# rehakvoj1/BIH-GPU-Raytracer

Measured on NVIDIA B200. Metric: Mrays/s, higher is better.
Workload: dtype f32

## Files before the change

bih-gpu-raytracer_b200/csrc/trace.cu:

```cuda
#include "bihrt_internal.cuh"
#include <float.h>

#define FULL 0xffffffffu
#define STACK_DEPTH_PARITY  32
#define STACK_DEPTH_QUALITY 96
#define NONE 0xFFFFFFFFu
#ifndef TRACE_THREADS
#define TRACE_THREADS 128
#endif
#ifndef TRACE_MIN_BLOCKS
#define TRACE_MIN_BLOCKS 8
#endif

#ifndef TRACE_COVERAGE_EXIT
#define TRACE_COVERAGE_EXIT 1
#endif
#define BOX_EPS 2.384185791015625e-07f

#define DET_EPS __uint_as_float(0x358637beu)

struct Hit { float t; int slot; };

__device__ __forceinline__ float fmin3(float a, float b, float c) { float r; asm("min.f32 %0, %1, %2, %3;" : "=f"(r) : "f"(a), "f"(b), "f"(c)); return r; }
__device__ __forceinline__ float fmax3(float a, float b, float c) { float r; asm("max.f32 %0, %1, %2, %3;" : "=f"(r) : "f"(a), "f"(b), "f"(c)); return r; }

__device__ __forceinline__ uint32_t pack_colour(uint32_t hits, int samples) {
    const float fh = (float)hits, fm = (float)(samples - (int)hits), fs = (float)samples;
    float cr = __fdiv_rn(__fadd_rn(__fmul_rn(fh, 255.f), __fmul_rn(fm, 20.f)), fs);
    float cb = __fdiv_rn(__fmul_rn(fm, 40.f), fs);
    cr = fmaxf(0.f, fminf(255.f, cr));
    cb = fmaxf(0.f, fminf(255.f, cb));
    return ((uint32_t)(int)cb << 16) | ((uint32_t)(int)cr << 8) | (uint32_t)(int)cr;
}

__device__ __forceinline__ float mt_det(float dx, float dy, float dz, float e1x, float e1y, float e1z, float e2x, float e2y, float e2z,
                                        float& px, float& py, float& pz) {
    px = __fsub_rn(__fmul_rn(dy, e2z), __fmul_rn(e2y, dz));
    py = __fsub_rn(__fmul_rn(dz, e2x), __fmul_rn(e2z, dx));
    pz = __fsub_rn(__fmul_rn(dx, e2y), __fmul_rn(e2x, dy));
    return __fadd_rn(__fadd_rn(__fmul_rn(e1x, px), __fmul_rn(e1y, py)), __fmul_rn(e1z, pz));
}
__device__ __forceinline__ float mt_u(float ox, float oy, float oz, const float4& q0, float px, float py, float pz, float inv,
                                      float& tx, float& ty, float& tz) {
    tx = __fsub_rn(ox, q0.x); ty = __fsub_rn(oy, q0.y); tz = __fsub_rn(oz, q0.z);
    return __fmul_rn(__fadd_rn(__fadd_rn(__fmul_rn(tx, px), __fmul_rn(ty, py)), __fmul_rn(tz, pz)), inv);
}
__device__ __forceinline__ float mt_v(float dx, float dy, float dz, float e1x, float e1y, float e1z, float tx, float ty, float tz, float inv,
                                      float& qx, float& qy, float& qz) {
    qx = __fsub_rn(__fmul_rn(ty, e1z), __fmul_rn(e1y, tz));
    qy = __fsub_rn(__fmul_rn(tz, e1x), __fmul_rn(e1z, tx));
    qz = __fsub_rn(__fmul_rn(tx, e1y), __fmul_rn(e1x, ty));
    return __fmul_rn(__fadd_rn(__fadd_rn(__fmul_rn(dx, qx), __fmul_rn(dy, qy)), __fmul_rn(dz, qz)), inv);
}

template <bool COUNTED, bool FIRST, bool RANGE = false, bool TWO_SIDED = false>
__device__ __forceinline__ void test_leaf(const char* __restrict__ first_tri, float ox, float oy, float oz,
                                          float dx, float dy, float dz, Hit& h, uint32_t& ntris, uint32_t& wleaf,
                                          const float* tlo_p = nullptr) {
    const float4* p = reinterpret_cast<const float4*>(first_tri);
    for (;;) {
        const float4 q0 = __ldg(p), q1 = __ldg(p + 1), q2 = __ldg(p + 2);
        if (COUNTED) { ntris++; const uint32_t am = __activemask(); wleaf += ((threadIdx.x & 31) == __ffs(am) - 1); }
        const float e1x = q0.w, e1y = q1.x, e1z = q1.y, e2x = q1.z, e2y = q1.w, e2z = q2.x;
        float px, py, pz;
        const float det = mt_det(dx, dy, dz, e1x, e1y, e1z, e2x, e2y, e2z, px, py, pz);
        if (!((TWO_SIDED ? fabsf(det) : det) < DET_EPS)) {
            const float inv = __frcp_rn(det);
            float tx, ty, tz;
            const float u = mt_u(ox, oy, oz, q0, px, py, pz, inv, tx, ty, tz);
            if (!(u < 0.f || u > 1.f)) {
                float qx, qy, qz;
                const float v = mt_v(dx, dy, dz, e1x, e1y, e1z, tx, ty, tz, inv, qx, qy, qz);
                if (!(v < 0.f || __fadd_rn(u, v) > 1.f)) {
                    const float t = __fmul_rn(__fadd_rn(__fadd_rn(__fmul_rn(e2x, qx), __fmul_rn(e2y, qy)), __fmul_rn(e2z, qz)), inv);
                    if (t > (RANGE ? *tlo_p : 0.f) && t < h.t) {
                        h.t = t; h.slot = (int)__float_as_uint(q2.w);
                        if (FIRST) break;
                    }
                }
            }
        }
        if (__float_as_uint(q2.z) & 1u) break;
        p += 3;
    }
}

template <int MODE, bool COUNTED, int WALK, bool Q>
__global__ void __launch_bounds__(TRACE_THREADS, TRACE_MIN_BLOCKS) k_trace(TraceArgs a) {
    constexpr int STACK_DEPTH = Q ? STACK_DEPTH_QUALITY : STACK_DEPTH_PARITY;
    constexpr bool COVER = MODE == 1 && TRACE_COVERAGE_EXIT != 0;
    constexpr bool LIST = MODE == 0 || MODE == 3 || MODE == 4;
    constexpr bool RANGE = MODE == 3 || MODE == 4;
    constexpr bool TWO_SIDED = MODE == 4;
    __shared__ __align__(16) float s_ray[TRACE_THREADS * 10];
    const int lane = threadIdx.x & 31;
    const uint32_t lt = (1u << lane) - 1u;
    float* my_ray = s_ray + threadIdx.x * 10;
    const char* __restrict__ nodes_b = reinterpret_cast<const char*>(a.nodes);
    const char* __restrict__ tris_b = reinterpret_cast<const char*>(a.tris);
    const BihTri* __restrict__ tris = a.tris;
    const uint32_t nu = a.hdr->nu;
    if (a.hdr->status != 0) return;
    if ((a.hdr->quality != 0) != Q) {
        if (blockIdx.x == 0 && threadIdx.x == 0 && a.status_map) *a.status_map = 0x100u;
        return;
    }
    const float blo[3] = { a.hdr->lo[0], a.hdr->lo[1], a.hdr->lo[2] }, bhi[3] = { a.hdr->hi[0], a.hdr->hi[1], a.hdr->hi[2] };
    uint32_t nnodes = 0, ntris = 0, maxsp = 0;
    uint32_t wnode = 0, wleaf = 0;

    uint64_t total;
    int tx = 1;
    if (LIST) total = a.tile_cost ? (((uint64_t)a.nrays + 1023u) >> 10) << 10 : (uint64_t)a.nrays;
    else {
        tx = (a.w + 31) / 32;
        const int ty = (a.h + 31) / 32, T = tx * ty;
        const int my_tiles = T > a.shard_index ? (T - a.shard_index + a.shard_count - 1) / a.shard_count : 0;
        total = ((uint64_t)my_tiles * 1024u) << a.gshift;
    }
    const int gshift = LIST ? 0 : a.gshift;
    const int nsamp = LIST ? 1 : ((a.s_end - a.s_begin) >> gshift);
    uint32_t my_queue = 0;
    if (a.queues > 1) { asm("mov.u32 %0, %%smid;" : "=r"(my_queue)); my_queue %= (uint32_t)a.queues; }
    uint64_t pool_next = 0, pool_end = 0;
    long long unit_t0 = 0; uint32_t unit_tile = 0xFFFFFFFFu;
    bool exhausted = false;

    uint64_t item = ~0ull;
    int s = 0, s0 = 0;
    uint32_t hits = 0, pixel = 0, pxy = 0;
    float ix = 1.f, iy = 1.f, iz = 1.f, nx = 0.f, ny = 0.f, nz = 0.f, bpad = 0.f;
    uint32_t cur = NONE;
    float rMin = 0.f, pMin = 0.f, pMax = 0.f;
    Hit h; h.t = FLT_MAX; h.slot = -1;
    bool tracing = false;
    uint4 stack[STACK_DEPTH];
    int sp = 0;
#define STACK_RESET() do { sp = 0; } while (0)
#define STACK_PUSH(item) do { stack[sp] = (item); sp++; } while (0)
#define STACK_POP(e) do { sp--; (e) = stack[sp]; } while (0)
    const uint32_t root_ref = BIH_REF_NODE(0, a.hdr->root_axis);
    const bool vote = WALK > 0 || a.vote_wait != 0;
    int thresh = a.refill_threshold;
    const bool direct = MODE == 1 && gshift > 0 && !(a.flags & BIHRT_RENDER_COUNTS);
    if (direct) thresh = 32;
    const int steps_per_vote = WALK > 0 ? WALK : (a.vote_walk > 0 ? a.vote_walk : 1);
    const uint32_t ray_smem = (uint32_t)__cvta_generic_to_shared(my_ray);

    for (;;) {
        const uint32_t idle = __ballot_sync(FULL, cur == NONE);
        const uint32_t busy = ~idle;
        if (idle && (busy == 0 || (thresh < 32 && __popc(__ballot_sync(FULL, cur == NONE && (tracing || item != ~0ull || LIST))) >= thresh))) {
            const bool fresh = (busy == 0);
            int new_thresh = -1;
            bool want_item = false, finishing = false;
            if (cur == NONE) {
                if (tracing) {
                    tracing = false;
                    if (MODE == 1) hits += (h.slot >= 0);
                    else if (RANGE) {
                        const bool hit = h.slot >= 0;
                        const bool rec = a.out_u || a.out_v || a.out_ng;
                        float u = 0.f, v = 0.f, gx = 0.f, gy = 0.f, gz = 0.f;
                        int32_t prim = -1;
                        if (hit && (rec || a.out_prim)) {
                            const float4* tq = reinterpret_cast<const float4*>(tris + h.slot);
                            const float4 q0 = __ldg(tq), q1 = __ldg(tq + 1), q2 = __ldg(tq + 2);
                            prim = (int32_t)__float_as_uint(q2.y);
                            if (rec) {
                                const float e1x = q0.w, e1y = q1.x, e1z = q1.y, e2x = q1.z, e2y = q1.w, e2z = q2.x;
                                const float2 dxy = *reinterpret_cast<const float2*>(my_ray + 6);
                                const float dx = dxy.x, dy = dxy.y, dz = my_ray[8];
                                float px, py, pz, tx, ty, tz, qx, qy, qz;
                                const float inv = __frcp_rn(mt_det(dx, dy, dz, e1x, e1y, e1z, e2x, e2y, e2z, px, py, pz));
                                u = mt_u(my_ray[0], my_ray[2], my_ray[4], q0, px, py, pz, inv, tx, ty, tz);
                                v = mt_v(dx, dy, dz, e1x, e1y, e1z, tx, ty, tz, inv, qx, qy, qz);
                                gx = __fsub_rn(__fmul_rn(e1y, e2z), __fmul_rn(e1z, e2y));
                                gy = __fsub_rn(__fmul_rn(e1z, e2x), __fmul_rn(e1x, e2z));
                                gz = __fsub_rn(__fmul_rn(e1x, e2y), __fmul_rn(e1y, e2x));
                            }
                        }
                        if (a.out_t) a.out_t[item] = hit ? h.t : FLT_MAX;
                        if (a.out_slot) a.out_slot[item] = h.slot;
                        if (a.out_prim) a.out_prim[item] = prim;
                        if (a.out_u) a.out_u[item] = u;
                        if (a.out_v) a.out_v[item] = v;
                        if (a.out_ng) { float* g = a.out_ng + 3 * item; g[0] = gx; g[1] = gy; g[2] = gz; }
                    } else {
                        const uint64_t o = MODE == 0 ? item : (uint64_t)pixel * (uint32_t)a.spp + (uint32_t)(s0 + s);
                        if (a.out_t) a.out_t[o] = h.t;
                        if (a.out_slot) a.out_slot[o] = h.slot;
                        if (a.out_prim) a.out_prim[o] = h.slot >= 0 ? (int32_t)tris[h.slot].prim : -1;
                    }
                    s++;
                    if (s == nsamp) {
                        if (MODE == 1 && gshift > 0) finishing = true;
                        else if (MODE == 1 && (a.flags & BIHRT_RENDER_COUNTS)) a.fb[pixel] = hits;
                        else if (MODE == 1) a.fb[pixel] = pack_colour(hits, nsamp);
                        item = ~0ull;
                    }
                }
                want_item = (item == ~0ull);
            }
            if (MODE == 1 && gshift > 0) {
                const uint32_t fin = __ballot_sync(FULL, finishing);
                if (finishing) {
                    const uint32_t same = __match_any_sync(fin, pixel);
                    const uint32_t sum = __reduce_add_sync(same, hits);
                    if (lane == __ffs(same) - 1) {
                        if (direct) a.fb[pixel] = pack_colour(sum, nsamp << gshift);
                        else if (sum) atomicAdd(&a.fb[pixel], sum);
                    }
                }
            }
            if (!LIST && fresh && a.tile_cost && unit_tile != 0xFFFFFFFFu) {
                if (lane == 0) atomicMax(a.tile_cost + unit_tile, (uint32_t)min((unsigned long long)(clock64() - unit_t0) >> 8, 0xFFFFFFFFull));
                unit_tile = 0xFFFFFFFFu;
            }
            uint32_t want = __ballot_sync(FULL, want_item);
            if (!LIST && busy != 0) want = 0;
            while (want && !exhausted) {
                if (pool_next >= pool_end) {
                    uint64_t base = ~0ull;
                    uint32_t got = 0;
                    if (lane == 0) {
                        const uint32_t ilc = (uint32_t)a.il_count, ili = (uint32_t)a.il_index, ics = (uint32_t)a.il_cshift;
                        if (a.queues <= 1) {
                            const uint32_t chunk = ilc > 1 ? 32u : (uint32_t)a.chunk_items;
                            const uint64_t fetched = atomicAdd(a.work, chunk); got = chunk;
                            const uint64_t lu = fetched >> 5;
                            base = ilc > 1 ? ((((lu >> ics) * ilc + ili) << ics) | (lu & ((1u << ics) - 1u))) << 5 : fetched;
                            if (base >= total) base = ~0ull;
                        } else {
                            const uint32_t tshift = 10 + gshift, ushift = 5 + gshift;
                            const uint64_t ntile = (total + ((1ull << tshift) - 1)) >> tshift;
                            for (uint32_t k = 0; k < (uint32_t)a.queues; k++) {
                                uint32_t q = my_queue + k; if (q >= (uint32_t)a.queues) q -= (uint32_t)a.queues;
                                if (q >= ntile) continue;
                                const uint32_t upt = (1u << ushift) / ilc;
                                const uint64_t units = ((ntile - q + a.queues - 1) / a.queues) * upt;
                                if (ld_relaxed(a.work + q) >= units) continue;
                                const uint32_t u = atomicAdd(a.work + q, 1u);
                                if (u >= units) continue;
                                const uint32_t lu = u % upt;
                                const uint64_t b = (((uint64_t)(u / upt) * a.queues + q) << tshift) + ((uint64_t)((((lu >> ics) * ilc + ili) << ics) | (lu & ((1u << ics) - 1u))) << 5);
                                if (b < total) { base = b; got = 32; break; }
                            }
                        }
                    }
                    base = __shfl_sync(FULL, base, 0);
                    got = __shfl_sync(FULL, got, 0);
                    if (LIST && a.tile_cost && unit_tile != 0xFFFFFFFFu) {
                        if (lane == 0) atomicMax(a.tile_cost + unit_tile, (uint32_t)min((unsigned long long)(clock64() - unit_t0) >> 8, 0xFFFFFFFFull));
                        unit_tile = 0xFFFFFFFFu;
                    }
                    if (base == ~0ull) { exhausted = true; break; }
                    pool_next = base;
                    pool_end = min(base + got, total);
                    if (a.tile_cost && unit_tile == 0xFFFFFFFFu) {
                        const uint32_t m = (uint32_t)(base >> (10 + gshift));
                        unit_tile = a.tile_order ? __ldg(a.tile_order + m) : m;
                        unit_t0 = clock64();
                    }
                }
                const uint64_t avail = pool_end - pool_next;
                const uint32_t rank = __popc(want & lt);
                const bool served = want_item && (uint64_t)rank < avail;
                if (served) {
                    item = pool_next + rank; s = 0; hits = 0; want_item = false;
                    if (LIST && a.tile_cost) {
                        const uint32_t mi = (uint32_t)(item >> 10);
                        const uint64_t ray = ((uint64_t)(a.tile_order ? __ldg(a.tile_order + mi) : mi) << 10) | (item & 1023u);
                        item = ray < (uint64_t)a.nrays ? ray : ~0ull;
                        if (item == ~0ull) want_item = true;
                    }
                    if (MODE == 0 && a.perm && item != ~0ull) item = __ldg(a.perm + item);
                    if (!LIST) {
                        const uint64_t pix = item >> gshift;
                        s0 = a.s_begin + (int)((uint32_t)item & ((1u << gshift) - 1u)) * nsamp;
                        const uint32_t mi = (uint32_t)(pix >> 10), q = (uint32_t)pix & 1023u;
                        const uint32_t m = a.tile_order ? __ldg(a.tile_order + mi) : mi;
                        const int tile = a.shard_index + (int)m * a.shard_count;
                        const int px = (tile % tx) * 32 + (int)((q >> 5) & 3u) * 8 + (int)(q & 7u);
                        const int py = (tile / tx) * 32 + (int)(q >> 7) * 4 + (int)((q >> 3) & 3u);
                        if (px < a.w && py < a.h) { pixel = (uint32_t)(py * a.w + px); pxy = (uint32_t)px | ((uint32_t)py << 16); }
                        else item = ~0ull;
                        if (item == ~0ull) want_item = true;
                    }
                }
                pool_next += min((uint64_t)__popc(want), avail);
                want = __ballot_sync(FULL, want_item);
            }
            if (cur == NONE && item != ~0ull) {
                float ox, oy, oz, dx, dy, dz;
                float tlo = 0.f, thi = FLT_MAX;
                bool live = true;
                if (RANGE) {
                    const float4* p = reinterpret_cast<const float4*>(a.rays_iv + item);
                    const float4 r0 = __ldg(p), r1 = __ldg(p + 1);
                    ox = r0.x; oy = r0.y; oz = r0.z; dx = r1.x; dy = r1.y; dz = r1.z;
                    tlo = fmaxf(r0.w, 0.f);
                    live = r0.w == r0.w && tlo < r1.w;
                    thi = fminf(r1.w, FLT_MAX);
                } else if (MODE == 0) {
                    const float* p = reinterpret_cast<const float*>(a.rays + item);
                    ox = __ldg(p); oy = __ldg(p + 1); oz = __ldg(p + 2); dx = __ldg(p + 3); dy = __ldg(p + 4); dz = __ldg(p + 5);
                } else {
                    const int px = (int)(pxy & 0xFFFFu), py = (int)(pxy >> 16);
                    const float ru = (a.flags & BIHRT_RENDER_JITTER) ? bihrt_jitter(a.seed, pixel, (uint32_t)(s0 + s), 0) : 0.5f;
                    const float rv = (a.flags & BIHRT_RENDER_JITTER) ? bihrt_jitter(a.seed, pixel, (uint32_t)(s0 + s), 1) : 0.5f;
                    const float uu = __fdiv_rn(__fadd_rn((float)px, ru), (float)a.w);
                    const float vv = __fdiv_rn(__fadd_rn((float)py, rv), (float)a.h);
                    ox = a.cam.origin[0]; oy = a.cam.origin[1]; oz = a.cam.origin[2];
                    dx = __fsub_rn(__fadd_rn(__fadd_rn(a.cam.lower_left[0], __fmul_rn(uu, a.cam.horizontal[0])), __fmul_rn(vv, a.cam.vertical[0])), ox);
                    dy = __fsub_rn(__fadd_rn(__fadd_rn(a.cam.lower_left[1], __fmul_rn(uu, a.cam.horizontal[1])), __fmul_rn(vv, a.cam.vertical[1])), oy);
                    dz = __fsub_rn(__fadd_rn(__fadd_rn(a.cam.lower_left[2], __fmul_rn(uu, a.cam.horizontal[2])), __fmul_rn(vv, a.cam.vertical[2])), oz);
                }
                ix = __frcp_rn(dx); iy = __frcp_rn(dy); iz = __frcp_rn(dz);
                nx = -__fmul_rn(ox, ix); ny = -__fmul_rn(oy, iy); nz = -__fmul_rn(oz, iz);
                bpad = __fmul_rn(BOX_EPS, fmaxf(fmaxf(fabsf(nx) <= FLT_MAX ? fabsf(nx) : 0.f, fabsf(ny) <= FLT_MAX ? fabsf(ny) : 0.f),
                                                fabsf(nz) <= FLT_MAX ? fabsf(nz) : 0.f));
                if (LIST && fresh) {
                    const uint32_t m = __activemask();
                    const uint32_t bx = __ballot_sync(m, ix < 0.f), by = __ballot_sync(m, iy < 0.f), bz = __ballot_sync(m, iz < 0.f);
                    const bool mixed = ((bx != 0 && bx != m) + (by != 0 && by != m) + (bz != 0 && bz != m)) >= 2;
                    new_thresh = mixed ? min(a.refill_threshold, a.refill_incoherent) : a.refill_threshold;
                }
                *reinterpret_cast<float2*>(my_ray) = make_float2(ox, ix); *reinterpret_cast<float2*>(my_ray + 2) = make_float2(oy, iy);
                *reinterpret_cast<float2*>(my_ray + 4) = make_float2(oz, iz); *reinterpret_cast<float2*>(my_ray + 6) = make_float2(dx, dy);
                my_ray[8] = dz;
                if (RANGE) my_ray[9] = tlo;
                h.t = RANGE ? thi : (MODE == 0 && a.any_hit) ? a.tmax : FLT_MAX; h.slot = -1; STACK_RESET(); tracing = true;
                bool in = nu > 0 && live;
                float tMin = __fmul_rn(__fsub_rn(ix < 0.f ? bhi[0] : blo[0], ox), ix);
                float tMax = __fmul_rn(__fsub_rn(ix < 0.f ? blo[0] : bhi[0], ox), ix);
                const float tymin = __fmul_rn(__fsub_rn(iy < 0.f ? bhi[1] : blo[1], oy), iy);
                const float tymax = __fmul_rn(__fsub_rn(iy < 0.f ? blo[1] : bhi[1], oy), iy);
                if ((tMin > tymax) || (tymin > tMax)) in = false;
                if (tymin > tMin) tMin = tymin;
                if (tymax < tMax) tMax = tymax;
                const float tzmin = __fmul_rn(__fsub_rn(iz < 0.f ? bhi[2] : blo[2], oz), iz);
                const float tzmax = __fmul_rn(__fsub_rn(iz < 0.f ? blo[2] : bhi[2], oz), iz);
                if ((tMin > tzmax) || (tzmin > tMax)) in = false;
                if (tzmin > tMin) tMin = tzmin;
                if (tzmax < tMax) tMax = tzmax;
                if (in) {
                    const float tabs = fmaxf(fabsf(tMin), fabsf(tMax));
                    bpad = __fmaf_rn(BOX_EPS, tabs <= FLT_MAX ? tabs : FLT_MAX, bpad);
                    const float qnan = __uint_as_float(0x7fc00000u);
                    ix = fabsf(ix) <= FLT_MAX ? ix : qnan; iy = fabsf(iy) <= FLT_MAX ? iy : qnan; iz = fabsf(iz) <= FLT_MAX ? iz : qnan;
                    rMin = tMin; pMin = fmaxf(tMin, tlo); pMax = ((MODE == 0 && a.any_hit) || COVER || RANGE) ? fminf(tMax, h.t) : tMax;
                    if (nu == 1) { cur = BIH_REF_LEAFREF(0); pMin = -FLT_MAX; pMax = FLT_MAX; }
                    else if (pMin <= pMax) cur = root_ref;
                }
            }
            if (LIST) {
                const uint32_t upd = __ballot_sync(FULL, new_thresh >= 0);
                if (upd) thresh = __shfl_sync(FULL, new_thresh, __ffs(upd) - 1);
            }
            if (__ballot_sync(FULL, cur != NONE || tracing) == 0 && exhausted &&
                __ballot_sync(FULL, item != ~0ull) == 0) break;
        }

#define BOX_SLAB(lx, ly, lz, hx, hy, hz, bn, bf)                                                            \
        do {                                                                                                \
            const float ax0 = __fmaf_rn((lx), ix, nx), ax1 = __fmaf_rn((hx), ix, nx);                       \
            const float ay0 = __fmaf_rn((ly), iy, ny), ay1 = __fmaf_rn((hy), iy, ny);                       \
            const float az0 = __fmaf_rn((lz), iz, nz), az1 = __fmaf_rn((hz), iz, nz);                       \
            const float n_ = fmaxf(fmaxf(fminf(ax0, ax1), fminf(ay0, ay1)), fminf(az0, az1));               \
            const float f_ = fminf(fminf(fmaxf(ax0, ax1), fmaxf(ay0, ay1)), fmaxf(az0, az1));               \
            (bn) = __fsub_rn(n_, bpad);                                                                     \
            (bf) = __fadd_rn(f_, bpad);                                                                     \
        } while (0)
#define POP_VALID()                                                                                         \
        do {                                                                                                \
            cur = NONE;                                                                                     \
            if (COVER) {                                   \
                if (sp > 0) {                                                                               \
                    uint4 e;                                                                                \
                    STACK_POP(e);                                                                           \
                    cur = e.x; rMin = __uint_as_float(e.y); pMin = __uint_as_float(e.z); pMax = __uint_as_float(e.w); \
                }                                                                                           \
            } else while (sp > 0) {                                                                         \
                uint4 e;                                                                                    \
                STACK_POP(e);                                                                               \
                const float m = fminf(__uint_as_float(e.w), h.t);                                           \
                if (__uint_as_float(e.z) <= m) { cur = e.x; rMin = __uint_as_float(e.y); pMin = __uint_as_float(e.z); pMax = m; break; } \
            }                                                                                               \
        } while (0)
        for (;;) {
#pragma unroll (WALK > 0 ? WALK : 1)
            for (int rep = 0; rep < steps_per_vote && (int)cur >= 0; rep++) {
                float2 oi;
                uint32_t ra;
                asm("mad.lo.u32 %0, %1, 8, %2;" : "=r"(ra) : "r"(cur & 3u), "r"(ray_smem));
                asm volatile("ld.shared.v2.f32 {%0, %1}, [%2];" : "=f"(oi.x), "=f"(oi.y) : "r"(ra));
                const float4* np;
                asm("mad.wide.u32 %0, %1, 64, %2;" : "=l"(np) : "r"(cur >> 2), "l"(nodes_b));
                float4 nd, b0, b1, b2;
                if (LIST) {
                    asm("ld.global.nc.v8.f32 {%0,%1,%2,%3,%4,%5,%6,%7}, [%8];"
                        : "=f"(nd.x), "=f"(nd.y), "=f"(nd.z), "=f"(nd.w), "=f"(b0.x), "=f"(b0.y), "=f"(b0.z), "=f"(b0.w) : "l"(np));
                    asm("ld.global.nc.v8.f32 {%0,%1,%2,%3,%4,%5,%6,%7}, [%8];"
                        : "=f"(b1.x), "=f"(b1.y), "=f"(b1.z), "=f"(b1.w), "=f"(b2.x), "=f"(b2.y), "=f"(b2.z), "=f"(b2.w) : "l"(np + 2));
                } else { nd = __ldg(np); b0 = __ldg(np + 1); b1 = __ldg(np + 2); b2 = __ldg(np + 3); }
                if (COUNTED) { nnodes++; const uint32_t am = __activemask(); wnode += (lane == __ffs(am) - 1); }
                const uint32_t rl = __float_as_uint(nd.z), rr = __float_as_uint(nd.w);
                const bool neg = oi.y < 0.f;
                const float t0 = __fmul_rn(__fsub_rn(nd.x, oi.x), oi.y);
                const float t1 = __fmul_rn(__fsub_rn(nd.y, oi.x), oi.y);
                const float tn = neg ? t1 : t0, tf = neg ? t0 : t1;
                const uint32_t refn = neg ? rr : rl, reff = neg ? rl : rr;
                float bnL, bfL, bnR, bfR;
                BOX_SLAB(b0.x, b0.y, b0.z, b0.w, b1.x, b1.y, bnL, bfL);
                BOX_SLAB(b1.z, b1.w, b2.x, b2.y, b2.z, b2.w, bnR, bfR);
                const float nLo = fmaxf(pMin, neg ? bnR : bnL), nHi = fmin3(pMax, tn, neg ? bfR : bfL);
                const float fLo = fmax3(pMin, tf, neg ? bnL : bnR), fHi = fminf(pMax, neg ? bfL : bfR);
                const bool go_near = (Q || rMin < tn) && (nLo <= nHi);
                const bool go_far = (fLo <= fHi);
                if (go_near && go_far) {
                    if ((int)refn >= 0 && (int)reff < 0) {
                        STACK_PUSH(make_uint4(refn, __float_as_uint(rMin), __float_as_uint(nLo), __float_as_uint(nHi)));
                        cur = reff; rMin = tf; pMin = fLo; pMax = fHi;
                    } else {
                        STACK_PUSH(make_uint4(reff, __float_as_uint(tf), __float_as_uint(fLo), __float_as_uint(fHi)));
                        cur = refn; pMin = nLo; pMax = nHi;
                    }
                    if (COUNTED) { maxsp = max(maxsp, (uint32_t)sp); if (sp >= STACK_DEPTH) { maxsp = 0x7fffffffu; sp = STACK_DEPTH - 1; } }
#ifdef BIHRT_DEBUG_STACK
                    if (sp >= STACK_DEPTH) __trap();
#endif
                } else if (go_near) { cur = refn; pMin = nLo; pMax = nHi; }
                else if (go_far) { cur = reff; rMin = tf; pMin = fLo; pMax = fHi; }
                else POP_VALID();
            }
            const uint32_t m_walk = __ballot_sync(FULL, (int)cur >= 0);
            if (m_walk == 0) break;
            if (vote) {
                const uint32_t m_wait = __ballot_sync(FULL, cur + 1u > 0x80000000u);
                if (__popc(m_wait) > __popc(m_walk)) break;
            }
        }
        if (cur + 1u > 0x80000000u) {
            const char* tp;
            asm("mad.wide.u32 %0, %1, 12, %2;" : "=l"(tp) : "r"(cur & 0x7FFFFFFCu), "l"(tris_b));
            const float2 dxy = *reinterpret_cast<const float2*>(my_ray + 6);
            test_leaf<COUNTED, COVER, RANGE, TWO_SIDED>(tp, my_ray[0], my_ray[2], my_ray[4], dxy.x, dxy.y, my_ray[8], h, ntris, wleaf, my_ray + 9);
            if (((LIST && a.any_hit) || COVER) && h.slot >= 0) { STACK_RESET(); cur = NONE; }
            else POP_VALID();
        }
#undef POP_VALID
#undef BOX_SLAB
#undef STACK_RESET
#undef STACK_PUSH
#undef STACK_POP
        __syncwarp();
    }

    if (COUNTED) {
#pragma unroll
        for (int o = 16; o > 0; o >>= 1) {
            nnodes += __shfl_xor_sync(FULL, nnodes, o);
            ntris += __shfl_xor_sync(FULL, ntris, o);
            maxsp = max(maxsp, __shfl_xor_sync(FULL, maxsp, o));
        }
        if (lane == 0) {
            atomicAdd(&a.counters[0], (unsigned long long)nnodes);
            atomicAdd(&a.counters[1], (unsigned long long)ntris);
            atomicMax(&a.counters[2], (unsigned long long)maxsp);
        }
        wnode = __reduce_add_sync(FULL, wnode); wleaf = __reduce_add_sync(FULL, wleaf);
        if (lane == 0) { atomicAdd(&a.counters[4], (unsigned long long)wnode); atomicAdd(&a.counters[5], (unsigned long long)wleaf); }
    }
}

__global__ void k_resolve(uint32_t* fb, int npix, int spp) {
    const int i = blockIdx.x * blockDim.x + threadIdx.x;
    if (i >= npix) return;
    fb[i] = pack_colour(fb[i], spp);
}

#define TILE_CLASSES 5
__device__ __forceinline__ int tile_class(uint32_t c, uint32_t mx) {
    int k = 0;
#pragma unroll
    for (int j = 1; j < TILE_CLASSES; j++) k += c < max(1u, mx >> j);
    return k;
}
__global__ void __launch_bounds__(1024) k_tile_order(uint32_t* __restrict__ cost, uint32_t* __restrict__ order, uint32_t ntiles) {
    __shared__ uint32_t s_w[TILE_CLASSES][32];
    __shared__ uint32_t s_max, s_base[TILE_CLASSES];
    const int lane = threadIdx.x & 31, w = threadIdx.x >> 5;
    const uint32_t per = (ntiles + 1023u) / 1024u, i0 = min(ntiles, threadIdx.x * per), i1 = min(ntiles, i0 + per);
    uint32_t mx = 0;
    for (uint32_t i = i0; i < i1; i++) mx = max(mx, cost[i]);
    mx = __reduce_max_sync(0xffffffffu, mx);
    if (lane == 0) s_w[0][w] = mx;
    __syncthreads();
    if (threadIdx.x == 0) { uint32_t m = 0; for (int k = 0; k < 32; k++) m = max(m, s_w[0][k]); s_max = m; }
    __syncthreads();
    mx = s_max;
    uint32_t cnt[TILE_CLASSES], inc[TILE_CLASSES];
#pragma unroll
    for (int k = 0; k < TILE_CLASSES; k++) cnt[k] = 0;
    for (uint32_t i = i0; i < i1; i++) {
        const int cl = tile_class(cost[i], mx);
#pragma unroll
        for (int k = 0; k < TILE_CLASSES; k++) cnt[k] += (cl == k);
    }
    __syncthreads();
#pragma unroll
    for (int k = 0; k < TILE_CLASSES; k++) {
        inc[k] = cnt[k];
#pragma unroll
        for (int o = 1; o < 32; o <<= 1) { const uint32_t t = __shfl_up_sync(0xffffffffu, inc[k], o); if (lane >= o) inc[k] += t; }
        if (lane == 31) s_w[k][w] = inc[k];
    }
    __syncthreads();
    if (threadIdx.x < TILE_CLASSES) {
        uint32_t run = 0;
        for (int j = 0; j < 32; j++) { const uint32_t x = s_w[threadIdx.x][j]; s_w[threadIdx.x][j] = run; run += x; }
        s_base[threadIdx.x] = run;
    }
    __syncthreads();
    if (threadIdx.x == 0) { uint32_t run = 0; for (int k = 0; k < TILE_CLASSES; k++) { const uint32_t x = s_base[k]; s_base[k] = run; run += x; } }
    __syncthreads();
    uint32_t pos[TILE_CLASSES];
#pragma unroll
    for (int k = 0; k < TILE_CLASSES; k++) pos[k] = s_base[k] + s_w[k][w] + inc[k] - cnt[k];
    for (uint32_t i = i0; i < i1; i++) {
        const int cl = tile_class(cost[i], mx);
#pragma unroll
        for (int k = 0; k < TILE_CLASSES; k++) if (cl == k) order[pos[k]++] = i;
    }
    __syncthreads();
    for (uint32_t i = i0; i < i1; i++) cost[i] = 0;
}

__global__ void __launch_bounds__(1024) k_tile_sort(uint32_t* __restrict__ cost, uint32_t* __restrict__ order, uint32_t ntiles) {
    __shared__ uint32_t s_cnt[256], s_off[256];
    if (threadIdx.x < 256) s_cnt[threadIdx.x] = 0;
    __syncthreads();
    for (uint32_t i = threadIdx.x; i < ntiles; i += 1024) atomicAdd(&s_cnt[min(255u, cost[i] >> 4)], 1u);
    __syncthreads();
    if (threadIdx.x == 0) { uint32_t run = 0; for (int b = 255; b >= 0; b--) { s_off[b] = run; run += s_cnt[b]; } }
    __syncthreads();
    for (uint32_t i = threadIdx.x; i < ntiles; i += 1024) order[atomicAdd(&s_off[min(255u, cost[i] >> 4)], 1u)] = i;
    __syncthreads();
    for (uint32_t i = threadIdx.x; i < ntiles; i += 1024) cost[i] = 0;
}

int bihrt_tile_order_launch(bihrt_ctx* c, uint32_t* cost, uint32_t* order, uint32_t ntiles, bool full_sort) {
    if (full_sort) k_tile_sort<<<1, 1024, 0, c->stream>>>(cost, order, ntiles);
    else k_tile_order<<<1, 1024, 0, c->stream>>>(cost, order, ntiles);
    c->kernel_launches += 1;
    BIHRT_CUDA(c, cudaGetLastError());
    return BIHRT_OK;
}

int bihrt_resolve_launch(bihrt_ctx* c, uint32_t* fb, int npix, int spp) {
    k_resolve<<<(npix + 255) / 256, 256, 0, c->stream>>>(fb, npix, spp);
    c->kernel_launches += 1;
    BIHRT_CUDA(c, cudaGetLastError());
    return BIHRT_OK;
}

#ifndef TRACE_WALK
#define TRACE_WALK 4
#endif
template <int MODE, bool COUNTED, int WALK, bool Q = false>
static int launch(bihrt_ctx* c, const TraceArgs& a) {
    int per_sm = c->opt_trace_blocks_per_sm;
    if (per_sm <= 0) {
        BIHRT_CUDA(c, cudaOccupancyMaxActiveBlocksPerMultiprocessor(&per_sm, k_trace<MODE, COUNTED, WALK, Q>, TRACE_THREADS, 0));
        if (per_sm < 1) per_sm = 1;
    }
    BIHRT_CUDA(c, cudaMemsetAsync(a.work, 0, 4 * 1024, c->stream));
    k_trace<MODE, COUNTED, WALK, Q><<<c->sm_count * per_sm, TRACE_THREADS, 0, c->stream>>>(a);
    c->kernel_launches += 1;
    BIHRT_CUDA(c, cudaGetLastError());
    return BIHRT_OK;
}

int bihrt_trace_launch(bihrt_ctx* c, const TraceArgs& a_in, int mode, bool counted) {
    TraceArgs a = a_in;
    const bool list = mode == 0 || mode == 3 || mode == 4;
    const int64_t rays = list ? a.nrays : (int64_t)a.w * a.h * (a.s_end - a.s_begin) / (a.shard_count > 0 ? a.shard_count : 1) / (a.il_count > 0 ? a.il_count : 1);
    const bool on = a.queues < 0 ? (rays >= (16ll << 20) && (list || a.gshift == 0)) : a.queues != 0;
    a.queues = on ? (c->sm_count < 1024 ? c->sm_count : 1024) : 1;
    uint32_t ntiles = 0;
    bihrt_ctx::TileKey key;
    if (!list) {
        const int tx = (a.w + 31) / 32, ty = (a.h + 31) / 32, T = tx * ty;
        const int mine = T > a.shard_index ? (T - a.shard_index + a.shard_count - 1) / a.shard_count : 0;
        if ((((uint64_t)mine * 1024u) << a.gshift) >= (1ull << 32) - (1ull << 24))
            return bihrt_fail(c, BIHRT_ERR_INVALID, "launch of %d tiles x 1024 pixels x %d lane groups exceeds the 32-bit work counter", mine, 1 << a.gshift);
    }
    const bool order_on = a.queues == 1 && (c->opt_tile_order > 1 || (c->opt_tile_order == 1 && rays >= (64ll << 10) && rays < (48ll << 20) && c->n >= 10000));
    if (order_on) {
        if (list) {
            if (a.nrays > 1024 && a.nrays <= (65536ll << 10)) { ntiles = (uint32_t)((a.nrays + 1023) >> 10); key.nrays = a.nrays; }
        } else {
            const int tx = (a.w + 31) / 32, ty = (a.h + 31) / 32, T = tx * ty;
            const int mine = T > a.shard_index ? (T - a.shard_index + a.shard_count - 1) / a.shard_count : 0;
            if (mine > 1 && mine <= 65536) ntiles = (uint32_t)mine;
            key.w = a.w; key.h = a.h; key.gshift = a.gshift; key.nsamp = a.s_end - a.s_begin; key.shard_index = a.shard_index;
            key.shard_count = a.shard_count; key.il_index = a.il_index; key.il_count = a.il_count; key.il_cshift = a.il_cshift;
        }
        key.mode = list ? mode : 1; key.ntiles = ntiles;
    }
    bihrt_ctx::TileSlot* slot = nullptr;
    if (ntiles) {
        for (auto& ts : c->tile_slots) if (ts.cap && ts.key == key) slot = &ts;
        if (!slot) {
            slot = &c->tile_slots[c->tile_next];
            c->tile_next = (c->tile_next + 1) % 4;
            slot->key = key; slot->valid = false;
        }
        if ((size_t)ntiles > slot->cap) {
            if (slot->cost) cudaFree(slot->cost);
            if (slot->order) cudaFree(slot->order);
            slot->cost = slot->order = nullptr; slot->cap = 0; slot->valid = false;
            if (cudaMalloc(&slot->cost, (size_t)ntiles * 4) != cudaSuccess || cudaMalloc(&slot->order, (size_t)ntiles * 4) != cudaSuccess) {
                cudaGetLastError();
                if (slot->cost) { cudaFree(slot->cost); slot->cost = nullptr; }
                slot = nullptr; ntiles = 0;
            } else slot->cap = ntiles;
        }
        if (slot) {
            if (!slot->valid) BIHRT_CUDA(c, cudaMemsetAsync(slot->cost, 0, (size_t)ntiles * 4, c->stream));
            a.tile_cost = slot->cost;
            a.tile_order = slot->valid ? slot->order : nullptr;
        }
    }
    const bool shipped = a.vote_wait != 0 && a.vote_walk == TRACE_WALK;
    int rc = BIHRT_ERR_INVALID;
    a.status_map = c->d_status_map;
    if (c->built_quality) {
        TraceArgs q = a; q.vote_wait = 1; q.vote_walk = 1;
        switch (mode * 2 + (counted ? 1 : 0)) {
            case 0: rc = launch<0, false, TRACE_WALK, true>(c, a); break;
            case 1: rc = launch<0, true, 0, true>(c, q); break;
            case 2: rc = launch<1, false, TRACE_WALK, true>(c, a); break;
            case 3: rc = launch<1, true, 0, true>(c, q); break;
            case 4: rc = launch<2, false, TRACE_WALK, true>(c, a); break;
            case 5: rc = launch<2, true, 0, true>(c, q); break;
            case 6: rc = launch<3, false, TRACE_WALK, true>(c, a); break;
            case 8: rc = launch<4, false, TRACE_WALK, true>(c, a); break;
            default: return bihrt_fail(c, BIHRT_ERR_INVALID, "bad trace mode %d", mode);
        }
    } else
    switch (mode * 2 + (counted ? 1 : 0)) {
        case 0: rc = shipped ? launch<0, false, TRACE_WALK>(c, a) : launch<0, false, 0>(c, a); break;
        case 1: rc = launch<0, true, 0>(c, a); break;
        case 2: rc = shipped ? launch<1, false, TRACE_WALK>(c, a) : launch<1, false, 0>(c, a); break;
        case 3: rc = launch<1, true, 0>(c, a); break;
        case 4: rc = shipped ? launch<2, false, TRACE_WALK>(c, a) : launch<2, false, 0>(c, a); break;
        case 5: rc = launch<2, true, 0>(c, a); break;
        case 6: rc = shipped ? launch<3, false, TRACE_WALK>(c, a) : launch<3, false, 0>(c, a); break;
        case 8: rc = shipped ? launch<4, false, TRACE_WALK>(c, a) : launch<4, false, 0>(c, a); break;
        default: return bihrt_fail(c, BIHRT_ERR_INVALID, "bad trace mode %d", mode);
    }
    if (rc == BIHRT_OK && slot) {
        if ((rc = bihrt_tile_order_launch(c, slot->cost, slot->order, ntiles, rays < c->opt_tile_sort_below)) == BIHRT_OK) slot->valid = true;
    }
    return rc;
}
```

Baseline: 13720.

## Specialize node traversal per warp-uniform ray octant in coverage mode

In coverage mode (MODE 1), each warp checks with ballots whether all its active rays share a direction-sign octant. It stores that octant in shared memory and then runs a node-walk loop instantiated for that octant. In the specialised loop the slab test picks near and far planes directly with 3-input min/max instead of per-axis min/max, which cuts ALU work per box. The cost is six extra ballots per refill, eight more copies of the traversal loop (more code and instruction-cache pressure), and a fallback path for warps with mixed octants.

```diff
diff --git a/bih-gpu-raytracer_b200/csrc/trace.cu b/bih-gpu-raytracer_b200/csrc/trace.cu
--- a/bih-gpu-raytracer_b200/csrc/trace.cu
+++ b/bih-gpu-raytracer_b200/csrc/trace.cu
@@ -15,6 +15,10 @@
 #ifndef TRACE_COVERAGE_EXIT
 #define TRACE_COVERAGE_EXIT 1
 #endif
+#ifndef TRACE_OCTANT_WALK
+#define TRACE_OCTANT_WALK 1
+#endif
+#define OCT_MIXED 8
 #define BOX_EPS 2.384185791015625e-07f
 
 #define DET_EPS __uint_as_float(0x358637beu)
@@ -89,6 +93,7 @@
 __global__ void __launch_bounds__(TRACE_THREADS, TRACE_MIN_BLOCKS) k_trace(TraceArgs a) {
     constexpr int STACK_DEPTH = Q ? STACK_DEPTH_QUALITY : STACK_DEPTH_PARITY;
     constexpr bool COVER = MODE == 1 && TRACE_COVERAGE_EXIT != 0;
+    constexpr bool OCTS = MODE == 1 && TRACE_OCTANT_WALK != 0;
     constexpr bool LIST = MODE == 0 || MODE == 3 || MODE == 4;
     constexpr bool RANGE = MODE == 3 || MODE == 4;
     constexpr bool TWO_SIDED = MODE == 4;
@@ -358,6 +363,17 @@
                 const uint32_t upd = __ballot_sync(FULL, new_thresh >= 0);
                 if (upd) thresh = __shfl_sync(FULL, new_thresh, __ffs(upd) - 1);
             }
+            if (OCTS) {
+                int oct = OCT_MIXED;
+                if (gshift > 0) {
+                    const bool w = cur != NONE;
+                    const uint32_t xn = __ballot_sync(FULL, w && ix < 0.f), xp = __ballot_sync(FULL, w && ix > 0.f);
+                    const uint32_t yn = __ballot_sync(FULL, w && iy < 0.f), yp = __ballot_sync(FULL, w && iy > 0.f);
+                    const uint32_t zn = __ballot_sync(FULL, w && iz < 0.f), zp = __ballot_sync(FULL, w && iz > 0.f);
+                    if (!((xn && xp) || (yn && yp) || (zn && zp))) oct = (xn != 0) | (yn != 0) << 1 | (zn != 0) << 2;
+                }
+                my_ray[9] = __int_as_float(oct);
+            }
             if (__ballot_sync(FULL, cur != NONE || tracing) == 0 && exhausted &&
                 __ballot_sync(FULL, item != ~0ull) == 0) break;
         }
@@ -367,8 +383,14 @@
             const float ax0 = __fmaf_rn((lx), ix, nx), ax1 = __fmaf_rn((hx), ix, nx);                       \
             const float ay0 = __fmaf_rn((ly), iy, ny), ay1 = __fmaf_rn((hy), iy, ny);                       \
             const float az0 = __fmaf_rn((lz), iz, nz), az1 = __fmaf_rn((hz), iz, nz);                       \
-            const float n_ = fmaxf(fmaxf(fminf(ax0, ax1), fminf(ay0, ay1)), fminf(az0, az1));               \
-            const float f_ = fminf(fminf(fmaxf(ax0, ax1), fmaxf(ay0, ay1)), fmaxf(az0, az1));               \
+            float n_, f_;                                                                                   \
+            if (OCT == OCT_MIXED) {                                                                         \
+                n_ = fmaxf(fmaxf(fminf(ax0, ax1), fminf(ay0, ay1)), fminf(az0, az1));                       \
+                f_ = fminf(fminf(fmaxf(ax0, ax1), fmaxf(ay0, ay1)), fmaxf(az0, az1));                       \
+            } else {                                             \
+                n_ = fmax3((OCT & 1) ? ax1 : ax0, (OCT & 2) ? ay1 : ay0, (OCT & 4) ? az1 : az0);            \
+                f_ = fmin3((OCT & 1) ? ax0 : ax1, (OCT & 2) ? ay0 : ay1, (OCT & 4) ? az0 : az1);            \
+            }                                                                                               \
             (bn) = __fsub_rn(n_, bpad);                                                                     \
             (bf) = __fadd_rn(f_, bpad);                                                                     \
         } while (0)
@@ -388,58 +410,97 @@
                 if (__uint_as_float(e.z) <= m) { cur = e.x; rMin = __uint_as_float(e.y); pMin = __uint_as_float(e.z); pMax = m; break; } \
             }                                                                                               \
         } while (0)
-        for (;;) {
-#pragma unroll (WALK > 0 ? WALK : 1)
-            for (int rep = 0; rep < steps_per_vote && (int)cur >= 0; rep++) {
-                float2 oi;
-                uint32_t ra;
-                asm("mad.lo.u32 %0, %1, 8, %2;" : "=r"(ra) : "r"(cur & 3u), "r"(ray_smem));
-                asm volatile("ld.shared.v2.f32 {%0, %1}, [%2];" : "=f"(oi.x), "=f"(oi.y) : "r"(ra));
-                const float4* np;
-                asm("mad.wide.u32 %0, %1, 64, %2;" : "=l"(np) : "r"(cur >> 2), "l"(nodes_b));
-                float4 nd, b0, b1, b2;
-                if (LIST) {
-                    asm("ld.global.nc.v8.f32 {%0,%1,%2,%3,%4,%5,%6,%7}, [%8];"
-                        : "=f"(nd.x), "=f"(nd.y), "=f"(nd.z), "=f"(nd.w), "=f"(b0.x), "=f"(b0.y), "=f"(b0.z), "=f"(b0.w) : "l"(np));
-                    asm("ld.global.nc.v8.f32 {%0,%1,%2,%3,%4,%5,%6,%7}, [%8];"
-                        : "=f"(b1.x), "=f"(b1.y), "=f"(b1.z), "=f"(b1.w), "=f"(b2.x), "=f"(b2.y), "=f"(b2.z), "=f"(b2.w) : "l"(np + 2));
-                } else { nd = __ldg(np); b0 = __ldg(np + 1); b1 = __ldg(np + 2); b2 = __ldg(np + 3); }
-                if (COUNTED) { nnodes++; const uint32_t am = __activemask(); wnode += (lane == __ffs(am) - 1); }
-                const uint32_t rl = __float_as_uint(nd.z), rr = __float_as_uint(nd.w);
-                const bool neg = oi.y < 0.f;
-                const float t0 = __fmul_rn(__fsub_rn(nd.x, oi.x), oi.y);
-                const float t1 = __fmul_rn(__fsub_rn(nd.y, oi.x), oi.y);
-                const float tn = neg ? t1 : t0, tf = neg ? t0 : t1;
-                const uint32_t refn = neg ? rr : rl, reff = neg ? rl : rr;
-                float bnL, bfL, bnR, bfR;
-                BOX_SLAB(b0.x, b0.y, b0.z, b0.w, b1.x, b1.y, bnL, bfL);
-                BOX_SLAB(b1.z, b1.w, b2.x, b2.y, b2.z, b2.w, bnR, bfR);
-                const float nLo = fmaxf(pMin, neg ? bnR : bnL), nHi = fmin3(pMax, tn, neg ? bfR : bfL);
-                const float fLo = fmax3(pMin, tf, neg ? bnL : bnR), fHi = fminf(pMax, neg ? bfL : bfR);
-                const bool go_near = (Q || rMin < tn) && (nLo <= nHi);
-                const bool go_far = (fLo <= fHi);
-                if (go_near && go_far) {
-                    if ((int)refn >= 0 && (int)reff < 0) {
-                        STACK_PUSH(make_uint4(refn, __float_as_uint(rMin), __float_as_uint(nLo), __float_as_uint(nHi)));
-                        cur = reff; rMin = tf; pMin = fLo; pMax = fHi;
-                    } else {
-                        STACK_PUSH(make_uint4(reff, __float_as_uint(tf), __float_as_uint(fLo), __float_as_uint(fHi)));
-                        cur = refn; pMin = nLo; pMax = nHi;
-                    }
-                    if (COUNTED) { maxsp = max(maxsp, (uint32_t)sp); if (sp >= STACK_DEPTH) { maxsp = 0x7fffffffu; sp = STACK_DEPTH - 1; } }
 #ifdef BIHRT_DEBUG_STACK
-                    if (sp >= STACK_DEPTH) __trap();
+#define DEBUG_STACK_TRAP() do { if (sp >= STACK_DEPTH) __trap(); } while (0)
+#else
+#define DEBUG_STACK_TRAP() do { } while (0)
 #endif
-                } else if (go_near) { cur = refn; pMin = nLo; pMax = nHi; }
-                else if (go_far) { cur = reff; rMin = tf; pMin = fLo; pMax = fHi; }
-                else POP_VALID();
-            }
-            const uint32_t m_walk = __ballot_sync(FULL, (int)cur >= 0);
-            if (m_walk == 0) break;
-            if (vote) {
-                const uint32_t m_wait = __ballot_sync(FULL, cur + 1u > 0x80000000u);
-                if (__popc(m_wait) > __popc(m_walk)) break;
-            }
+#define NODE_PHASE(OCT_)                                                                                           \
+        do {                                                                                                        \
+            constexpr int OCT = (OCT_);                                                                             \
+            for (;;) {                                                                                              \
+                _Pragma("unroll (WALK > 0 ? WALK : 1)")                                                             \
+                for (int rep = 0; rep < steps_per_vote && (int)cur >= 0; rep++) {                                   \
+                                    \
+                    float2 oi;                                                                                      \
+                    uint32_t ra;                                                                                    \
+                    asm("mad.lo.u32 %0, %1, 8, %2;" : "=r"(ra) : "r"(cur & 3u), "r"(ray_smem));                     \
+                    asm volatile("ld.shared.v2.f32 {%0, %1}, [%2];" : "=f"(oi.x), "=f"(oi.y) : "r"(ra));            \
+                           \
+                    const float4* np;                                                                               \
+                    asm("mad.wide.u32 %0, %1, 64, %2;" : "=l"(np) : "r"(cur >> 2), "l"(nodes_b));                   \
+                     \
+                     \
+                     \
+                     \
+                     \
+                                                                          \
+                    float4 nd, b0, b1, b2;                                                                          \
+                    if (LIST) {                                                                                     \
+                        asm("ld.global.nc.v8.f32 {%0,%1,%2,%3,%4,%5,%6,%7}, [%8];"                                  \
+                            : "=f"(nd.x), "=f"(nd.y), "=f"(nd.z), "=f"(nd.w), "=f"(b0.x), "=f"(b0.y), "=f"(b0.z), "=f"(b0.w) : "l"(np)); \
+                        asm("ld.global.nc.v8.f32 {%0,%1,%2,%3,%4,%5,%6,%7}, [%8];"                                  \
+                            : "=f"(b1.x), "=f"(b1.y), "=f"(b1.z), "=f"(b1.w), "=f"(b2.x), "=f"(b2.y), "=f"(b2.z), "=f"(b2.w) : "l"(np + 2)); \
+                    } else { nd = __ldg(np); b0 = __ldg(np + 1); b1 = __ldg(np + 2); b2 = __ldg(np + 3); }          \
+                    if (COUNTED) { nnodes++; const uint32_t am = __activemask(); wnode += (lane == __ffs(am) - 1); } \
+                    const uint32_t rl = __float_as_uint(nd.z), rr = __float_as_uint(nd.w);                          \
+                    const bool neg = oi.y < 0.f;                                       \
+                    const float t0 = __fmul_rn(__fsub_rn(nd.x, oi.x), oi.y);                          \
+                    const float t1 = __fmul_rn(__fsub_rn(nd.y, oi.x), oi.y);                                        \
+                    const float tn = neg ? t1 : t0, tf = neg ? t0 : t1;                                             \
+                    const uint32_t refn = neg ? rr : rl, reff = neg ? rl : rr;                                      \
+                     \
+                     \
+                     \
+                     \
+                                                              \
+                    float bnL, bfL, bnR, bfR;                                                                       \
+                    BOX_SLAB(b0.x, b0.y, b0.z, b0.w, b1.x, b1.y, bnL, bfL);                                         \
+                    BOX_SLAB(b1.z, b1.w, b2.x, b2.y, b2.z, b2.w, bnR, bfR);                                         \
+                     \
+                    const float nLo = fmaxf(pMin, neg ? bnR : bnL), nHi = fmin3(pMax, tn, neg ? bfR : bfL);         \
+                    const float fLo = fmax3(pMin, tf, neg ? bnL : bnR), fHi = fminf(pMax, neg ? bfL : bfR);         \
+                    const bool go_near = (Q || rMin < tn) && (nLo <= nHi);    \
+                    const bool go_far = (fLo <= fHi);                                                               \
+                     \
+                          \
+                    if (go_near && go_far) {                                                                        \
+                             \
+                        if ((int)refn >= 0 && (int)reff < 0) {                                                      \
+                            STACK_PUSH(make_uint4(refn, __float_as_uint(rMin), __float_as_uint(nLo), __float_as_uint(nHi))); \
+                            cur = reff; rMin = tf; pMin = fLo; pMax = fHi;                                          \
+                        } else {                                                                                    \
+                            STACK_PUSH(make_uint4(reff, __float_as_uint(tf), __float_as_uint(fLo), __float_as_uint(fHi))); \
+                            cur = refn; pMin = nLo; pMax = nHi;                                                     \
+                        }                                                                                           \
+                         \
+                         \
+                                                           \
+                        if (COUNTED) { maxsp = max(maxsp, (uint32_t)sp); if (sp >= STACK_DEPTH) { maxsp = 0x7fffffffu; sp = STACK_DEPTH - 1; } } \
+                        DEBUG_STACK_TRAP();                                                                         \
+                    } else if (go_near) { cur = refn; pMin = nLo; pMax = nHi; }                                     \
+                    else if (go_far) { cur = reff; rMin = tf; pMin = fLo; pMax = fHi; }                             \
+                    else POP_VALID();                                                                               \
+                }                                                                                                   \
+                const uint32_t m_walk = __ballot_sync(FULL, (int)cur >= 0);                                         \
+                if (m_walk == 0) break;                                                                             \
+                if (vote) {                                                                                         \
+                    const uint32_t m_wait = __ballot_sync(FULL, cur + 1u > 0x80000000u);   \
+                    if (__popc(m_wait) > __popc(m_walk)) break;                                                     \
+                }                                                                                                   \
+            }                                                                                                       \
+        } while (0)
+        if constexpr (!OCTS) NODE_PHASE(OCT_MIXED);
+        else switch (__float_as_int(my_ray[9])) {
+            case 0: NODE_PHASE(0); break;
+            case 1: NODE_PHASE(1); break;
+            case 2: NODE_PHASE(2); break;
+            case 3: NODE_PHASE(3); break;
+            case 4: NODE_PHASE(4); break;
+            case 5: NODE_PHASE(5); break;
+            case 6: NODE_PHASE(6); break;
+            case 7: NODE_PHASE(7); break;
+            default: NODE_PHASE(OCT_MIXED); break;
         }
         if (cur + 1u > 0x80000000u) {
             const char* tp;
@@ -449,6 +510,8 @@
             if (((LIST && a.any_hit) || COVER) && h.slot >= 0) { STACK_RESET(); cur = NONE; }
             else POP_VALID();
         }
+#undef NODE_PHASE
+#undef DEBUG_STACK_TRAP
 #undef POP_VALID
 #undef BOX_SLAB
 #undef STACK_RESET
```

New measurement: 14650, median of 6. 6.7% higher.
